# Plonky3/Plonky3-recursion

Hardware: AMD Instinct MI355X
Metric: prove_next_layer ms + Poseidon2 perms/s, KoalaBear 2^20-row circuit, 1/8 GPU (lower is better)
Workload: dtype u32 Montgomery (31-bit prime field, degree-4 extension); Poseidon2 hashing as exact integers in f64; 1 GPU; prove_next_layer (verifier-circuit run on the device + prove_all_tables) of the synthetic koala-bear 2^20-row recursion layer: tables const/public/alu/poseidon2/recompose, FRI blowup 4, arity<=4, 54 queries, 15-bit PoW; circuit inputs + NextLayerPrepCache resident in HBM; field=koala-bear, log_height=20, independent_proofs=1, proof_bytes=612900, parallelism=1 independent proofs, one per GPU, no data-path collective

## Files before the change

plonky3_recursion_amd/csrc/context.h:

```cpp
#pragma once
#include <hip/hip_runtime.h>

#include <algorithm>
#include <array>
#include <atomic>
#include <cstdarg>
#include <cstdio>
#include <cstring>
#include <exception>
#include <functional>
#include <map>
#include <memory>
#include <chrono>
#include <mutex>
#include <stdexcept>
#include <string>
#include <thread>
#include <tuple>
#include <vector>

#include "../../include/p3r.h"
#include "field.h"
#include "poseidon2.h"
#include "proof_layout.h"
// ... 298 lines not shown
  void end_proof() { in_proof = false; }
  HostPost() = default;
  HostPost(const HostPost&) = delete;
  HostPost& operator=(const HostPost&) = delete;
  ~HostPost() {
    if (host) (void)hipHostFree(host);
  }
  hipError_t post(hipStream_t s, const uint32_t* src, size_t words, const uint32_t** out) {
    if (!host) {
      hipError_t e = hipHostMalloc(reinterpret_cast<void**>(&host), (kWords + 16) * 4,
                                   hipHostMallocMapped | hipHostMallocCoherent);
      if (e != hipSuccess) return e;
      e = hipHostGetDevicePointer(reinterpret_cast<void**>(&dev), host, 0);
      if (e != hipSuccess) {
        (void)hipHostFree(host);
        host = nullptr;
        dev = nullptr;
        return e;
      }
      host[kWords] = 0;
    }
    *out = host;
    ++seq;
    hipLaunchKernelGGL(k_post_small, dim3(1), dim3(256), 0, s, dev, src, (uint32_t)words, dev + kWords, seq);
    hipError_t e = hipGetLastError();
    if (e != hipSuccess) return e;
    volatile uint32_t* flag = host + kWords;
    const int sl = slot < kSlots ? slot : kSlots - 1;
    if (in_proof) ++slot;
    const auto t0 = std::chrono::steady_clock::now();
    auto elapsed_ns = [&] { return (int64_t)std::chrono::duration_cast<std::chrono::nanoseconds>(std::chrono::steady_clock::now() - t0).count(); };
    const int64_t expect = in_proof ? expect_ns[sl] : 0;
    if (expect > 400000) {
      const int64_t until = expect - std::max<int64_t>(expect / 4, 200000);
      for (int64_t now = elapsed_ns(); now < until && *flag != seq; now = elapsed_ns())
        std::this_thread::sleep_for(std::chrono::nanoseconds(std::min<int64_t>(until - now, 500000)));
    }
    const int64_t awake_until = expect > 400000 ? expect + expect / 2 + 500000 : 0;
    for (uint64_t spins = 0;; ++spins) {
      if (*flag == seq) break;
      if (spins > (uint64_t(1) << 14) && (spins & 0x3F) == 0x3F) {
        if (awake_until && elapsed_ns() < awake_until) std::this_thread::yield();
        else if (spins > (uint64_t(1) << 17)) std::this_thread::sleep_for(std::chrono::microseconds(20));
        else std::this_thread::yield();
      }
      if ((spins & 0xFFF) == 0xFFF) {
        e = hipStreamQuery(s);
        if (e != hipErrorNotReady) {
          if (e != hipSuccess) return e;
          if (*flag == seq) break;
          return hipStreamSynchronize(s);
        }
      }
    }
    if (in_proof) expect_ns[sl] = elapsed_ns();
    std::atomic_thread_fence(std::memory_order_acquire);
    return hipSuccess;
  }
};

struct DevBuf {
  uint32_t* p = nullptr;
  size_t n = 0;
  std::shared_ptr<DevPool> pool;
  DevBuf() = default;
  explicit DevBuf(size_t cells) { alloc(cells); }
  DevBuf(const DevBuf&) = delete;
  DevBuf& operator=(const DevBuf&) = delete;
  DevBuf(DevBuf&& o) noexcept : p(o.p), n(o.n), pool(std::move(o.pool)) { o.p = nullptr; o.n = 0; }
  DevBuf& operator=(DevBuf&& o) noexcept {
    if (this != &o) { release(); p = o.p; n = o.n; pool = std::move(o.pool); o.p = nullptr; o.n = 0; }
    return *this;
  }
  ~DevBuf() { release(); }
  void alloc(size_t cells) {
    release();
    if (cells) {
      pool = tls_pool();
      if (!pool) fail(P3R_EINVAL, "device allocation outside a p3r API call");
      p = static_cast<uint32_t*>(pool->get(cells * sizeof(uint32_t)));
    }
    n = cells;
  }
  void release() {
    if (p) pool->put(p, n * sizeof(uint32_t));
    p = nullptr;
    n = 0;
    pool.reset();
  }
};

inline int log2_exact(size_t x, const char* what) {
  if (x == 0 || (x & (x - 1))) fail(P3R_EINVAL, "%s (%zu) must be a power of two", what, x);
  int l = 0;
  while ((size_t(1) << l) < x) ++l;
  return l;
}

}

struct p3r_dmat {
  p3r::DevBuf buf;
  uint32_t* d = nullptr;
  size_t h = 0, w = 0;
};

struct p3r_p2_dev {
  size_t n = 0;
  std::unique_ptr<p3r_dmat> inputs;
  p3r::DevBuf flags;
  p3r::DevBuf seed;
};

struct p3r_tree {
  std::vector<const p3r_dmat*> mats;
  std::vector<std::unique_ptr<p3r_dmat>> owned;
  int salt_elems = 0;
  std::vector<std::unique_ptr<p3r_dmat>> salt_owned;
  p3r::DevBuf phase_salts;
  size_t phase_salt_stride = 0, phase_rows = 0;
  int log_max_h = 0;
  int cap_height = 0;
  size_t total_width = 0;
  std::vector<p3r::DevBuf> layers;
  int arity = 2;
  std::vector<p3r::MmcsLevel> levels;
  std::vector<size_t> layer_n;
};

namespace p3r {
struct ProfRec {
  const char* name;
  hipEvent_t a, b;
};
}

struct p3r_ctx {
  p3r_config cfg{};
  std::shared_ptr<p3r::DevPool> pool = std::make_shared<p3r::DevPool>();
  bool prof_enabled = false;
  std::vector<p3r::ProfRec> prof;
  std::vector<std::pair<std::string, double>> stage_ms;
  std::string cur_stage;
  double cur_stage_t0 = 0;
  int partial_rounds = 0;
  hipStream_t stream = nullptr;
  int n_cus = 256;
  p3r::DevBuf rc;
  p3r::DevBuf rc_f64;
  const double* rcd() const { return reinterpret_cast<const double*>(rc_f64.p); }
  size_t rcd_w32_at = 0;
  const double* rcd_w32() const { return rcd() + rcd_w32_at; }
  p3r::DevBuf p2_diag;
  std::vector<uint32_t> rc_canonical;
  std::vector<uint8_t> fri_log_arities;
  p3r::ProofLayout proof_layout;
  std::vector<uint32_t> rc_mont_host;
  std::string err;
  bool w32_diag_builtin = false;
  bool w32_unacknowledged = false;
  uint64_t zk_nonce = 0;
  uint32_t zk_key[8] = {0, 0, 0, 0, 0, 0, 0, 0};
  std::vector<uint8_t> pending_proof;
  p3r::HostStage stage;
  p3r::HostLanding landing;
  p3r::HostPost post;
  std::map<std::string, p3r::DevBuf> const_tables;

  std::map<std::pair<int, int>, p3r::DevBuf> tw_sub;
  std::map<std::pair<int, int>, std::pair<p3r::DevBuf, p3r::DevBuf>> tw4;
  std::map<std::tuple<int, int, uint32_t>, std::pair<p3r::DevBuf, p3r::DevBuf>> pre;
  std::map<std::pair<int, uint32_t>, std::pair<p3r::DevBuf, p3r::DevBuf>> inv_pow;
};

inline hipError_t fetch_small(p3r_ctx* ctx, const uint32_t* src, size_t words, uint32_t* dst) {
  if (words == 0) return hipSuccess;
  if (words <= p3r::HostPost::kWords) {
    const uint32_t* got = nullptr;
    p3r::host_mark("fetch: posted, waiting for the GPU");
    hipError_t e = ctx->post.post(ctx->stream, src, words, &got);
    p3r::host_mark("fetch: arrived");
    if (e != hipSuccess) return e;
    std::memcpy(dst, got, words * 4);
    return hipSuccess;
  }
  return p3r::copy_sync(ctx->stream, dst, src, words * 4, hipMemcpyDeviceToHost);
}
```

plonky3_recursion_amd/csrc/kernels_coop.hip.h:

```cpp
#pragma once
#include "kernels.hip.h"

namespace p3r {

template <int CTRL>
__device__ __forceinline__ uint32_t dpp(uint32_t v) {
  return (uint32_t)__builtin_amdgcn_update_dpp(0, (int)v, CTRL, 0xF, 0xF, false);
}
constexpr int DPP_QUAD_NEXT1 = 0x39;
constexpr int DPP_QUAD_NEXT2 = 0x4E;
constexpr int DPP_QUAD_NEXT3 = 0x93;
constexpr int DPP_ROW_ROR1 = 0x121, DPP_ROW_ROR2 = 0x122, DPP_ROW_ROR4 = 0x124, DPP_ROW_ROR8 = 0x128;

template <class F>
__device__ __forceinline__ F coop_external(F x) {
  F b = F::raw(dpp<DPP_QUAD_NEXT1>(x.v)), c = F::raw(dpp<DPP_QUAD_NEXT2>(x.v)), d = F::raw(dpp<DPP_QUAD_NEXT3>(x.v));
  F ab = x + b;
  F y = ab.dbl() + b + (c + d);
  F t = y + F::raw(dpp<DPP_ROW_ROR4>(y.v));
  t = t + F::raw(dpp<DPP_ROW_ROR8>(t.v));
  return y + t;
}
template <class F>
__device__ __forceinline__ F coop_row_sum(F x) {
  F t = x + F::raw(dpp<DPP_ROW_ROR8>(x.v));
  t = t + F::raw(dpp<DPP_ROW_ROR4>(t.v));
  t = t + F::raw(dpp<DPP_ROW_ROR2>(t.v));
  return t + F::raw(dpp<DPP_ROW_ROR1>(t.v));
}

constexpr int DPP_QUAD_BCAST0 = 0x00;
__device__ __forceinline__ uint32_t coop_bcast0(uint32_t x0) {
  uint32_t q = dpp<DPP_QUAD_BCAST0>(x0);
  q |= dpp<DPP_ROW_ROR4>(q);
  return q | dpp<DPP_ROW_ROR8>(q);
}

template <class PP>
struct CoopRc {
  uint32_t full[2 * P2_HALF_FULL];
  uint32_t part[PP::PARTIAL_ROUNDS];
};
template <class PP>
__device__ __forceinline__ CoopRc<PP> coop_load_rc(const uint32_t* __restrict__ rc, int elem) {
  CoopRc<PP> c;
#pragma unroll
  for (int r = 0; r < P2_HALF_FULL; ++r) c.full[r] = rc[r * P2_WIDTH + elem];
#pragma unroll
  for (int r = 0; r < PP::PARTIAL_ROUNDS; ++r) c.part[r] = rc[P2_HALF_FULL * P2_WIDTH + r];
#pragma unroll
  for (int r = 0; r < P2_HALF_FULL; ++r)
    c.full[P2_HALF_FULL + r] = rc[P2_HALF_FULL * P2_WIDTH + PP::PARTIAL_ROUNDS + r * P2_WIDTH + elem];
  return c;
}

template <class PP>
__device__ __forceinline__ Fp<PP> coop_permute(Fp<PP> s, int elem, Fp<PP> diag, const CoopRc<PP>& rc) {
  using F = Fp<PP>;
  s = coop_external(s);
#pragma unroll
  for (int r = 0; r < P2_HALF_FULL; ++r) {
    s = p2_sbox<PP>(s + F::raw(rc.full[r]));
    s = coop_external(s);
  }
#pragma unroll
  for (int r = 0; r < PP::PARTIAL_ROUNDS; ++r) {
    const F rest = coop_row_sum(elem == 0 ? F::zero() : s);
    const F sb = p2_sbox<PP>(s + F::raw(rc.part[r]));
    const F sum = rest + F::raw(coop_bcast0(elem == 0 ? sb.v : 0u));
    s = (elem == 0 ? sb : s) * diag + sum;
  }
#pragma unroll
  for (int r = 0; r < P2_HALF_FULL; ++r) {
    s = p2_sbox<PP>(s + F::raw(rc.full[P2_HALF_FULL + r]));
    s = coop_external(s);
  }
  return s;
}

template <class PP>
__global__ void __launch_bounds__(kBlock)
k_mmcs_hash_rows_strided_coop(const uint32_t* const* __restrict__ cols, int wtot, size_t h, size_t stride,
                              uint32_t* __restrict__ dig, const uint32_t* __restrict__ rc,
                              const uint32_t* __restrict__ diag) {
  using F = Fp<PP>;
  const size_t gid = (size_t)blockIdx.x * kBlock + threadIdx.x;
  const size_t row = gid >> 4;
  const int e = (int)(gid & 15);
  const bool live = row < h;
  const F d = F::raw(diag[e]);
  const CoopRc<PP> rcs = coop_load_rc<PP>(rc, e);
  F s = F::zero();
  for (int g = 0; g < wtot; g += P2_RATE) {
    if (live && e < P2_RATE && g + e < wtot) s = F::raw(cols[g + e][row * stride]);
    s = coop_permute<PP>(s, e, d, rcs);
  }
  if (live && e < P2_DIGEST) dig[(size_t)e * h + row] = s.v;
}

constexpr int kSubtreeBlock = 1024;
constexpr int kSubtreeNodes = 256;
constexpr int kSubtreeLevels = 8;
struct SubtreeArgs {
  const uint32_t* in;
  uint32_t n_in;
  uint32_t local;
  int n_levels;
  uint32_t* out[kSubtreeLevels];
  const uint32_t* inj[kSubtreeLevels];
  uint32_t* t_state;
  uint32_t* t_beta;
  uint32_t* t_cap;
  int t_dc;
};

template <class PP>
__device__ __forceinline__ void fri_transcript_step(int j, uint32_t root_word, uint32_t* __restrict__ state,
                                                    uint32_t* __restrict__ beta_out, uint32_t* __restrict__ cap_out,
                                                    const CoopRc<PP>& rc, const uint32_t* __restrict__ diag, int dc = 4) {
  using F = Fp<PP>;
  F s = j < P2_RATE ? F::raw(root_word) : F::raw(state[j]);
  if (j < P2_RATE) cap_out[j] = s.v;
  if (j == P2_RATE) s += F::from_canonical(P2_RATE);
  s = coop_permute<PP>(s, j, F::raw(diag[j]), rc);
  state[j] = s.v;
  if (j >= P2_RATE - dc && j < P2_RATE) beta_out[7 - j] = s.v;
}
template <class PP>
__global__ void __launch_bounds__(kSubtreeBlock)
k_mmcs_subtree(SubtreeArgs a, const uint32_t* __restrict__ rc, const uint32_t* __restrict__ diag) {
  using F = Fp<PP>;
  __shared__ uint32_t buf[2][P2_DIGEST * kSubtreeNodes / 2];
  const int elem = threadIdx.x & 15;
  const uint32_t group = threadIdx.x >> 4, k = elem & 7;
  const F d = F::raw(diag[elem]);
  const CoopRc<PP> rcs = coop_load_rc<PP>(rc, elem);
  uint32_t n = a.n_in < a.local ? a.n_in : a.local;
  uint32_t n_glob = a.n_in, first = blockIdx.x * n;
#pragma unroll
  for (int l = 0; l < kSubtreeLevels; ++l) {
    if (l < a.n_levels) {
      const uint32_t nn = n / 2, nn_glob = n_glob / 2, first_out = first / 2;
      const uint32_t* cur = buf[(l + 1) & 1];
      uint32_t* nxt = buf[l & 1];
      for (uint32_t node = group; node < nn; node += blockDim.x / 16) {
        const uint32_t child = 2 * node + (elem >> 3);
        F s = F::raw(l == 0 ? a.in[(size_t)k * n_glob + first + child] : cur[k * n + child]);
        s = coop_permute<PP>(s, elem, d, rcs);
        if (a.inj[l]) {
          if (elem >= P2_DIGEST) s = F::raw(a.inj[l][(size_t)k * nn_glob + first_out + node]);
          s = coop_permute<PP>(s, elem, d, rcs);
        }
        if (elem < P2_DIGEST) {
          nxt[k * nn + node] = s.v;
          a.out[l][(size_t)k * nn_glob + first_out + node] = s.v;
        }
      }
      __syncthreads();
      n = nn;
      n_glob = nn_glob;
      first = first_out;
    }
  }
  if (a.t_state && threadIdx.x < P2_WIDTH) {
    const uint32_t* root = buf[(a.n_levels - 1) & 1];
    fri_transcript_step<PP>((int)threadIdx.x, threadIdx.x < P2_RATE ? root[threadIdx.x] : 0u, a.t_state, a.t_beta,
                            a.t_cap, rcs, diag, a.t_dc ? a.t_dc : 4);
  }
}

template <class PP>
__global__ void __launch_bounds__(64)
k_fri_transcript_step(const uint32_t* __restrict__ root , uint32_t* __restrict__ state ,
                      uint32_t* __restrict__ beta_out , uint32_t* __restrict__ cap_out ,
                      const uint32_t* __restrict__ rc, const uint32_t* __restrict__ diag, int dc) {
  const int j = threadIdx.x;
  if (j >= P2_WIDTH) return;
  fri_transcript_step<PP>(j, j < P2_RATE ? root[j] : 0u, state, beta_out, cap_out, coop_load_rc<PP>(rc, j), diag, dc);
}



template <class F>
__device__ __forceinline__ F coop32_pair_sum(F t) {
  const auto r = __builtin_amdgcn_permlane16_swap(t.v, t.v, false, false);
  return F::raw(r[0]) + F::raw(r[1]);
}
template <class F>
__device__ __forceinline__ F coop32_external(F x) {
  const F b = F::raw(dpp<DPP_QUAD_NEXT1>(x.v)), c = F::raw(dpp<DPP_QUAD_NEXT2>(x.v)), d = F::raw(dpp<DPP_QUAD_NEXT3>(x.v));
  const F ab = x + b;
  const F y = ab.dbl() + b + (c + d);
  F t = y + F::raw(dpp<DPP_ROW_ROR4>(y.v));
  t = t + F::raw(dpp<DPP_ROW_ROR8>(t.v));
  return y + coop32_pair_sum(t);
}
template <class F>
__device__ __forceinline__ F coop32_sum(F x) { return coop32_pair_sum(coop_row_sum(x)); }
__device__ __forceinline__ uint32_t coop32_bcast0(uint32_t x0) {
  const uint32_t q = coop_bcast0(x0);
  const auto r = __builtin_amdgcn_permlane16_swap(q, q, false, false);
  return r[0] | r[1];
}

template <class PP>
struct Coop32Rc {
  uint32_t full[2 * P2_HALF_FULL];
  uint32_t part[PP::PARTIAL_ROUNDS_W32];
  uint32_t diag;
};
template <class PP>
__device__ __forceinline__ Coop32Rc<PP> coop32_load_rc(const uint32_t* __restrict__ rcw, int elem) {
  Coop32Rc<PP> c;
#pragma unroll
  for (int r = 0; r < P2_HALF_FULL; ++r) c.full[r] = rcw[r * P2W_WIDTH + elem];
#pragma unroll
  for (int r = 0; r < PP::PARTIAL_ROUNDS_W32; ++r) c.part[r] = rcw[P2_HALF_FULL * P2W_WIDTH + r];
#pragma unroll
  for (int r = 0; r < P2_HALF_FULL; ++r)
    c.full[P2_HALF_FULL + r] = rcw[P2_HALF_FULL * P2W_WIDTH + PP::PARTIAL_ROUNDS_W32 + r * P2W_WIDTH + elem];
  c.diag = rcw[p2w_num_rc<PP>() + elem];
  return c;
}
template <class PP>
__device__ __forceinline__ Fp<PP> coop32_permute(Fp<PP> s, int elem, const Coop32Rc<PP>& rc) {
  using F = Fp<PP>;
  const F diag = F::raw(rc.diag);
  s = coop32_external(s);
#pragma unroll
  for (int r = 0; r < P2_HALF_FULL; ++r) {
    s = p2_sbox<PP>(s + F::raw(rc.full[r]));
    s = coop32_external(s);
  }
#pragma unroll 1
  for (int r = 0; r < PP::PARTIAL_ROUNDS_W32; ++r) {
    const F rest = coop32_sum(elem == 0 ? F::zero() : s);
    const F sb = p2_sbox<PP>(s + F::raw(rc.part[r]));
    const F sum = rest + F::raw(coop32_bcast0(elem == 0 ? sb.v : 0u));
    s = (elem == 0 ? sb : s) * diag + sum;
  }
#pragma unroll
  for (int r = 0; r < P2_HALF_FULL; ++r) {
    s = p2_sbox<PP>(s + F::raw(rc.full[P2_HALF_FULL + r]));
    s = coop32_external(s);
  }
  return s;
}

}
```

plonky3_recursion_amd/csrc/mmcs_impl.hip.h:

```cpp

namespace {

template <class PP>
void hash_rows(p3r_ctx* ctx, const std::vector<std::vector<const p3r_dmat*>>& classes,
               const std::vector<uint32_t*>& digs) {
  std::vector<HashRowsJob> jobs;
  for (size_t c = 0; c < classes.size(); ++c) {
    std::vector<const uint32_t*> cols;
    for (const p3r_dmat* m : classes[c])
      for (size_t k = 0; k < m->w; ++k) cols.push_back(m->d + k * m->h);
    HashRowsJob j{};
    j.cols = col_table(ctx, cols);
    j.dig = digs[c];
    j.h = classes[c][0]->h;
    j.wtot = (int)cols.size();
    jobs.push_back(j);
  }
  std::stable_sort(jobs.begin(), jobs.end(),
                   [](const HashRowsJob& a, const HashRowsJob& b) { return a.wtot > b.wtot; });
  uint32_t blocks = 0;
  double perms = 0;
  for (auto& j : jobs) {
    j.block0 = blocks;
    blocks += blocks_for(j.h);
    perms += (double)j.h * ((j.wtot + P2_RATE - 1) / P2_RATE);
  }
  prof_count(ctx, "hash_rows_perms", perms);
  const auto* d_jobs =
      static_cast<const HashRowsJob*>(const_table(ctx, jobs.data(), jobs.size() * sizeof(HashRowsJob)));
  ProfScope ps(ctx, "mmcs_hash_rows");
  hipLaunchKernelGGL(k_mmcs_hash_rows<PP>, dim3(blocks), dim3(kBlock), 0, ctx->stream, d_jobs, (int)jobs.size(),
                     ctx->rcd());
  P3R_HIP(hipGetLastError());
}

inline size_t env_pow2(const char* name, size_t dflt, size_t lo, size_t hi) {
  const char* e = tuning_knob(name);
  size_t v = e ? (size_t)atol(e) : dflt;
  v = std::min(std::max(v, lo), hi);
  while (v & (v - 1)) v &= v - 1;
  return v;
}
inline size_t coop_max_nodes() {
  static const size_t v = env_pow2("P3R_COOP_MAX_NODES", 16384, 1, size_t(1) << 30);
  return v;
}
inline size_t coop_max_leaf_rows() {
  static const size_t v = env_pow2("P3R_COOP_MAX_LEAF_ROWS", 8192, 1, size_t(1) << 30);
  return v;
}
inline size_t subtree_nodes() {
  static const size_t v = env_pow2("P3R_SUBTREE_NODES", 32, 2, kSubtreeNodes);
  return v;
}
template <class PP>
void launch_compress(p3r_ctx* ctx, const uint32_t* prev, const uint32_t* inj, uint32_t* out, size_t n) {
  ProfScope ps(ctx, "mmcs_compress");
  hipLaunchKernelGGL(k_mmcs_compress<PP>, dim3(blocks_for(n)), dim3(kBlock), 0, ctx->stream, prev, inj, out, n,
                     ctx->rcd());
  P3R_HIP(hipGetLastError());
}

using InjectMap = std::map<size_t, DevBuf>;
inline const uint32_t* injected_at(const InjectMap* inject, const MmcsLevel& lv) {
  if (!lv.inject_h) return nullptr;
  if (!inject || !inject->count(lv.inject_h) || lv.inject_h != lv.logical_next)
    fail(P3R_EINVAL, "MMCS: matrix heights must be powers of two");
  return inject->at(lv.inject_h).p;
}
inline void push_layer(p3r_tree* tree, size_t n) {
  tree->layers.emplace_back(P2_DIGEST * n);
  tree->layer_n.push_back(n);
}

struct TranscriptStep {
  uint32_t *state, *beta, *cap;
  bool done = false;
  int dc = 4;
};
template <class PP>
size_t mmcs_subtree(p3r_ctx* ctx, p3r_tree* tree, size_t l, const InjectMap* inject, TranscriptStep* step) {
  const size_t n = tree->layer_n.back();
  if (n / 2 > coop_max_nodes()) return 0;
  SubtreeArgs a{};
  a.in = tree->layers.back().p;
  a.n_in = (uint32_t)n;
  const size_t local = std::min<size_t>(n, subtree_nodes());
  a.local = (uint32_t)local;
  for (size_t shrink = local; shrink > 1 && l + a.n_levels < tree->levels.size() && a.n_levels < kSubtreeLevels; shrink /= 2) {
    const MmcsLevel& lv = tree->levels[l + a.n_levels];
    push_layer(tree, lv.padded_next);
    a.out[a.n_levels] = tree->layers.back().p;
    a.inj[a.n_levels] = injected_at(inject, lv);
    ++a.n_levels;
  }
  if (step && tree->layer_n.back() == 1 && n == local) {
    a.t_state = step->state;
    a.t_beta = step->beta;
    a.t_cap = step->cap;
    a.t_dc = step->dc;
    step->done = true;
  }
  ProfScope ps(ctx, "mmcs_compress");
  const unsigned lanes = (unsigned)std::min<size_t>(std::max<size_t>(local * 8, 64), kSubtreeBlock);
  hipLaunchKernelGGL(k_mmcs_subtree<PP>, dim3((unsigned)(n / local)), dim3(lanes), 0, ctx->stream, a,
                     ctx->rc.p, ctx->p2_diag.p);
  P3R_HIP(hipGetLastError());
  return (size_t)a.n_levels;
}

inline void mmcs_begin(p3r_ctx* ctx, p3r_tree* tree, const std::vector<size_t>& heights) {
  const size_t hmax = *std::max_element(heights.begin(), heights.end());
  tree->arity = ctx->cfg.mmcs_arity == 4 ? 4 : 2;
  tree->log_max_h = log2_exact(hmax, "matrix height");
  tree->cap_height = (int)ctx->cfg.cap_height;
  tree->levels = tree->arity == 4 ? mmcs4_schedule(heights) : mmcs2_schedule(heights, tree->log_max_h, tree->cap_height);
  tree->layers.clear();
  tree->layer_n.clear();
  const size_t n0 = tree->arity == 4 ? mmcs4_padded_len(hmax) : hmax;
  push_layer(tree, n0);
  if (n0 != hmax) P3R_HIP(fill_async(ctx->stream, tree->layers[0].p, 0, P2_DIGEST * n0 * 4));
}

template <class PP>
void mmcs_build_levels(p3r_ctx* ctx, p3r_tree* tree, const InjectMap* inject, TranscriptStep* step = nullptr) {
  for (size_t l = 0; l < tree->levels.size();) {
    if (tree->arity != 4) {
      const size_t built = mmcs_subtree<PP>(ctx, tree, l, inject, step);
      if (built) {
        l += built;
        continue;
      }
    }
    const MmcsLevel& lv = tree->levels[l++];
    DevBuf next(P2_DIGEST * lv.padded_next);
    const uint32_t* inj = injected_at(inject, lv);
    if (tree->arity == 4)
      mmcs4_compress<PP>(ctx, tree->layers.back().p, tree->layer_n.back(), lv.step, inj, next.p, lv.logical_next, lv.padded_next);
    else
      launch_compress<PP>(ctx, tree->layers.back().p, inj, next.p, lv.padded_next);
    tree->layers.push_back(std::move(next));
    tree->layer_n.push_back(lv.padded_next);
  }
}

template <class PP>
void mmcs_hash_rows_strided(p3r_ctx* ctx, p3r_tree* tree, const std::vector<const uint32_t*>& cols, size_t rows, size_t stride) {
  const uint32_t* const* dcols = col_table(ctx, cols);
  uint32_t* dig = tree->layers[0].p;
  if (tree->arity == 4) {
    mmcs4_hash_rows_strided<PP>(ctx, dcols, (int)cols.size(), rows, stride, dig, tree->layer_n[0]);
  } else {
    ProfScope ps(ctx, "mmcs_hash_rows_strided");
    if (rows <= coop_max_leaf_rows())
      hipLaunchKernelGGL(k_mmcs_hash_rows_strided_coop<PP>, dim3(blocks_for(rows * 16)), dim3(kBlock), 0,
                         ctx->stream, dcols, (int)cols.size(), rows, stride, dig, ctx->rc.p, ctx->p2_diag.p);
    else
      hipLaunchKernelGGL(k_mmcs_hash_rows_strided<PP>, dim3(blocks_for(rows)), dim3(kBlock), 0, ctx->stream,
                         dcols, (int)cols.size(), rows, stride, dig, ctx->rcd());
  }
  P3R_HIP(hipGetLastError());
}

inline std::vector<uint32_t> mmcs_cap_mont(p3r_ctx* ctx, const p3r_tree* tree) {
  const size_t cap_n = tree->layer_n.back();
  std::vector<uint32_t> soa(P2_DIGEST * cap_n), cap(P2_DIGEST * cap_n);
  P3R_HIP(fetch_small(ctx, tree->layers.back().p, soa.size(), soa.data()));
  for (size_t j = 0; j < cap_n; ++j)
    for (int k = 0; k < P2_DIGEST; ++k) cap[j * P2_DIGEST + k] = soa[(size_t)k * cap_n + j];
  return cap;
}

template <class PP>
std::vector<uint32_t> mmcs_commit(p3r_ctx* ctx, p3r_tree* tree) {
  const auto& mats = tree->mats;
  if (mats.empty()) fail(P3R_EINVAL, "MMCS commit needs at least one matrix");
  std::vector<size_t> order(mats.size()), heights, class_h;
  std::iota(order.begin(), order.end(), 0);
  std::stable_sort(order.begin(), order.end(),
                   [&](size_t a, size_t b) { return mats[a]->h > mats[b]->h; });
  const size_t hmax = mats[order[0]]->h;
  const int log_max_h = log2_exact(hmax, "matrix height");
  if ((int)ctx->cfg.cap_height > log_max_h)
    fail(P3R_EINVAL, "cap_height %d exceeds log2 of the tallest matrix (%d)", (int)ctx->cfg.cap_height, log_max_h);
  tree->total_width = 0;
  for (auto* m : mats) {
    tree->total_width += m->w;
    heights.push_back(m->h);
  }
  mmcs_begin(ctx, tree, heights);
  for (size_t i : order)
    if (class_h.empty() || class_h.back() != mats[i]->h) class_h.push_back(mats[i]->h);
  InjectMap inject;
  {
    std::vector<std::vector<const p3r_dmat*>> classes;
    std::vector<uint32_t*> digs;
    std::vector<size_t> allocs;
    for (size_t h : class_h) {
      std::vector<const p3r_dmat*> v;
      for (size_t i : order)
        if (mats[i]->h == h) v.push_back(mats[i]);
      classes.push_back(std::move(v));
      digs.push_back(h == hmax ? tree->layers[0].p : inject.emplace(h, DevBuf(P2_DIGEST * h)).first->second.p);
      allocs.push_back(h == hmax ? tree->layer_n[0] : h);
    }
    if (tree->arity == 4) mmcs4_hash_rows<PP>(ctx, classes, digs, allocs);
    else hash_rows<PP>(ctx, classes, digs);
  }
  mmcs_build_levels<PP>(ctx, tree, &inject);
  return mmcs_cap_mont(ctx, tree);
}

template <class PP>
void mmcs_open(p3r_ctx* ctx, const p3r_tree* tree, size_t index, uint32_t* opened, uint32_t* proof) {
  using F = Fp<PP>;
  if (index >> tree->log_max_h) fail(P3R_EINVAL, "open index %zu out of range", index);
  size_t off = 0;
  for (const p3r_dmat* m : tree->mats) {
    int lh = log2_exact(m->h, "matrix height");
    size_t row = index >> (tree->log_max_h - lh);
    P3R_HIP(hipMemcpy2DAsync(opened + off, 4, m->d + row, m->h * 4, 4, m->w, hipMemcpyDeviceToHost,
                             ctx->stream));
    off += m->w;
  }
  size_t depth = 0;
  for (size_t l = 0; l < tree->levels.size(); ++l) {
    const size_t step = tree->levels[l].step, idx = index >> tree->levels[l].bits, pos = idx & (step - 1);
    for (size_t j = 0; j < step; ++j) {
      if (j == pos) continue;
      P3R_HIP(hipMemcpy2DAsync(proof + depth * P2_DIGEST, 4, tree->layers[l].p + (idx - pos + j), tree->layer_n[l] * 4, 4,
                               P2_DIGEST, hipMemcpyDeviceToHost, ctx->stream));
      ++depth;
    }
  }
  P3R_HIP(hipStreamSynchronize(ctx->stream));
  for (size_t i = 0; i < off; ++i) opened[i] = F::raw(opened[i]).to_canonical();
  for (size_t i = 0; i < depth * P2_DIGEST; ++i) proof[i] = F::raw(proof[i]).to_canonical();
}

struct OpenItem {
  const uint32_t* base;
  uint64_t n;
  uint32_t dst;
  uint32_t shift;
  uint32_t step, slot;
};
template <class PP>
__global__ void __launch_bounds__(256)
k_mmcs_open_batch(const OpenItem* __restrict__ items, uint32_t n_items, const uint32_t* __restrict__ indices, uint32_t words,
// ... 72 lines not shown
```

plonky3_recursion_amd/csrc/p3r_core.hip:

```cpp
#include "context.h"
#include "kernels.hip.h"
#include "kernels_stark.hip.h"
#include "kernels_coop.hip.h"
#include "tu_api.h"
#include "profile.h"
#include "run_schedule.h"
#include "prep_device.h"
#include "host_abi.h"

#include <sys/random.h>

#include <algorithm>
#include <cerrno>
#include <future>
#include <numeric>
#include <unordered_map>

using namespace p3r;

namespace {

thread_local std::string g_create_error;

template <class Fn>
// ... 136 lines not shown
  hipLaunchKernelGGL(k_p2w_permute_rows<PP>, dim3(blocks_for(n)), dim3(kBlock), 0, ctx->stream, d, n, ctx->rc.p + p2_num_constants<PP>());
  P3R_HIP(hipGetLastError());
}

template <class PP>
std::unique_ptr<p3r_dmat> coset_lde(p3r_ctx* ctx, const p3r_dmat* in, int added_bits, uint32_t shift) {
  return std::move(coset_lde_batch<PP>(ctx, {{in, shift}}, added_bits)[0]);
}

template <class PP>
void init_ctx(p3r_ctx* ctx) {
  using F = Fp<PP>;
  const size_t nrc = p2_num_constants<PP>();
  const std::vector<uint32_t> table = constants_table<PP>(ctx->cfg, [](const char* what, uint32_t got, size_t want) {
    fail(P3R_EINVAL, "%s is %u, the field needs %zu constants", what, got, want);
  });
  const uint32_t* src = table.data();
  ctx->rc_canonical = table;
  std::vector<uint32_t> mont(table.size());
  for (size_t i = 0; i < table.size(); ++i) {
    if (table[i] >= PP::P) fail(P3R_EINVAL, "permutation constant %zu is not canonical", i);
    mont[i] = F::from_canonical(table[i]).v;
  }
  ctx->rc_mont_host = mont;
  ctx->rc.alloc(mont.size());
  P3R_HIP(copy_sync(ctx->stream, ctx->rc.p, mont.data(), mont.size() * 4, hipMemcpyHostToDevice));
  std::vector<double> rcd(src, src + nrc);
  ctx->rcd_w32_at = nrc;
  {
    const size_t nrcw = p2w_num_rc<PP>();
    const uint32_t* w = src + nrc;
    rcd.insert(rcd.end(), w, w + nrcw);
    for (int i = 0; i < P2W_WIDTH; ++i) {
      const uint32_t d = w[nrcw + i];
      rcd.push_back(d > PP::P / 2 ? (double)d - (double)PP::P : (double)d);
    }
    const uint32_t* builtin = PP::FIELD_ID == 0 ? kDefaultDiagW32_koala_bear : kDefaultDiagW32_baby_bear;
    const bool is_builtin = std::equal(builtin, builtin + P2W_WIDTH, w + nrcw) && !tuning_knob("P3R_W32_GENERAL_DIAG");
    ctx->w32_diag_builtin = is_builtin;
  }
  ctx->rc_f64.alloc(2 * rcd.size());
  P3R_HIP(copy_sync(ctx->stream, ctx->rc_f64.p, rcd.data(), rcd.size() * 8, hipMemcpyHostToDevice));
  {
    auto inv2k = [](int k) { return F::from_u64(uint64_t(1) << k).inv(); };
    const F two = F::from_canonical(2), three = F::from_canonical(3), four = F::from_canonical(4);
    F d[16] = {-two, F::one(), two, inv2k(1), three, four, -inv2k(1), -three, -four, inv2k(8), inv2k(3), inv2k(24),
               -inv2k(8), -inv2k(3), -inv2k(4), -inv2k(24)};
    if (PP::FIELD_ID == 1) {
      F b[16] = {-two, F::one(), two, inv2k(1), three, four, -inv2k(1), -three, -four, inv2k(8), inv2k(2), inv2k(3),
                 inv2k(27), -inv2k(8), -inv2k(4), -inv2k(27)};
      for (int i = 0; i < 16; ++i) d[i] = b[i];
    }
    uint32_t dm[16];
    for (int i = 0; i < 16; ++i) dm[i] = d[i].v;
    ctx->p2_diag.alloc(16);
    P3R_HIP(copy_sync(ctx->stream, ctx->p2_diag.p, dm, sizeof dm, hipMemcpyHostToDevice));
  }
  ctx->partial_rounds = PP::PARTIAL_ROUNDS;
  ctx->cfg.poseidon2_rc = nullptr;
  ctx->w32_unacknowledged = (!ctx->cfg.poseidon2_w32_rc || !ctx->cfg.poseidon2_w32_diag) && !(ctx->cfg.ext_choices & P3R_EXT_UNPINNED_W32_DEFAULTS);
  if (ctx->w32_unacknowledged && ctx->cfg.mmcs_arity == 4)
    fail(P3R_EINVAL, "mmcs_arity = 4 with poseidon2_w32_rc / poseidon2_w32_diag NULL: the built-in width-32 constants are self-generated, "
                     "not upstream's - pass the caller's, or acknowledge with P3R_EXT_UNPINNED_W32_DEFAULTS");
  ctx->cfg.poseidon2_w32_rc = nullptr;
  ctx->cfg.poseidon2_w32_diag = nullptr;
  if (ctx->cfg.fri_log_arities) ctx->fri_log_arities.assign(ctx->cfg.fri_log_arities, ctx->cfg.fri_log_arities + ctx->cfg.fri_log_arities_len);
  ctx->cfg.fri_log_arities = nullptr;
  if (!ctx->proof_layout.set(ctx->cfg.proof_layout, ctx->cfg.proof_layout_len))
    fail(P3R_EINVAL, "proof_layout must be 18 bytes: three permutations batch[5] | fri[5] | opened[8]");
  ctx->cfg.proof_layout = nullptr;
  lde_init<PP>(ctx);
}

}

#include "mmcs_impl.hip.h"
#include "prove_impl.hip.h"
#include "layer_impl.hip.h"
#include "circuit_impl.hip.h"

namespace {
template <class PP>
void mmcs_commit_canonical(p3r_ctx* ctx, p3r_tree* tree, uint32_t* cap_out) {
  const size_t S = ctx->cfg.mmcs_salt_elems, n_mats = tree->mats.size();
  if (S) {
    const std::vector<const p3r_dmat*> mats = tree->mats;
    for (const p3r_dmat* m : mats) log2_exact(m->h, "matrix height");
    const ZkKey key = zk_key_of(ctx, ctx->zk_nonce++);
    tree->salt_elems = (int)S;
    tree->salt_owned = draw_salts<PP>(ctx, mats, kSaltRound + ZK_ROUND_PUBLIC_COMMIT, key);
    tree->mats.clear();
    for (size_t i = 0; i < n_mats; ++i) { tree->mats.push_back(mats[i]); tree->mats.push_back(tree->salt_owned[i].get()); }
  }
  const std::vector<uint32_t> cap = mmcs_commit<PP>(ctx, tree);
  tree->total_width -= n_mats * S;
  for (size_t i = 0; i < cap.size(); ++i) cap_out[i] = Fp<PP>::raw(cap[i]).to_canonical();
}
}

extern "C" {

p3r_ctx* p3r_create(const p3r_config* cfg) {
  p3r_ctx* ctx = nullptr;
  int rc = guard(nullptr, [&] {
    if (!cfg) fail(P3R_EINVAL, "cfg is NULL");
    if (cfg->abi_version != P3R_ABI_VERSION)
      fail(P3R_EINVAL, "abi_version %u != %u", cfg->abi_version, P3R_ABI_VERSION);
    if (cfg->field != P3R_FIELD_KOALA_BEAR && cfg->field != P3R_FIELD_BABY_BEAR)
      fail(P3R_EUNSUPPORTED, "unsupported field id %u", cfg->field);
    if (cfg->mmcs_arity != 0 && cfg->mmcs_arity != 2 && cfg->mmcs_arity != 4)
      fail(P3R_EINVAL, "mmcs_arity must be 2 or 4 (got %u)", cfg->mmcs_arity);
    if (cfg->mmcs_arity == 4 && cfg->cap_height != 0) fail(P3R_EUNSUPPORTED, "arity-4 MMCS: cap_height must be 0");
    if (cfg->zk > 1) fail(P3R_EINVAL, "zk must be 0 or 1 (got %u)", cfg->zk);
    if (cfg->zk && cfg->num_random_codewords > 8) fail(P3R_EINVAL, "num_random_codewords must be in 1..8 (0 selects 2)");
    if (cfg->challenge_degree != 0 && cfg->challenge_degree != 4 &&
        !(cfg->challenge_degree == 5 && cfg->field == P3R_FIELD_KOALA_BEAR))
      fail(P3R_EUNSUPPORTED, "UnsupportedChallengeDegree(%u): 4, or 5 over KoalaBear", cfg->challenge_degree);
    if (p3r::ext_degree_is_binomial_generic(cfg->ext_degree)) {
      const uint32_t P = cfg->field == P3R_FIELD_KOALA_BEAR ? p3r::KoalaBearParams::P : p3r::BabyBearParams::P;
      if (cfg->ext_w == 0 || cfg->ext_w >= P) fail(P3R_EINVAL, "MissingWForExtension: ext_degree %u needs ext_w in 1..p-1", cfg->ext_degree);
    } else if (cfg->ext_degree != 1 && cfg->ext_degree != 4 && !(cfg->ext_degree == 5 && cfg->field == P3R_FIELD_KOALA_BEAR))
      fail(P3R_EUNSUPPORTED, "UnsupportedExtDegree(%u): 1, 2, 4, 6, 8, or 5 over KoalaBear", cfg->ext_degree);
    int ndev = 0;
    hipError_t e = hipGetDeviceCount(&ndev);
    if (e != hipSuccess || ndev == 0)
      fail(P3R_ENODEV, "no HIP device available (%s); this library has no CPU fallback",
           e == hipSuccess ? "device count is 0" : hipGetErrorString(e));
    if (cfg->device < 0 || cfg->device >= ndev)
      fail(P3R_ENODEV, "device %d out of range (%d devices)", cfg->device, ndev);
    P3R_HIP(hipSetDevice(cfg->device));
    auto c = std::make_unique<p3r_ctx>();
    c->cfg = *cfg;
    tls_pool() = c->pool;
    P3R_HIP(hipStreamCreateWithFlags(&c->stream, hipStreamNonBlocking));
    {
      int cus = 0;
      if (hipDeviceGetAttribute(&cus, hipDeviceAttributeMultiprocessorCount, cfg->device) == hipSuccess && cus > 0) c->n_cus = cus;
    }
    if (cfg->mmcs_salt_elems > 16) fail(P3R_EINVAL, "mmcs_salt_elems must be in 0..16 (got %u)", cfg->mmcs_salt_elems);
    if (cfg->zk || cfg->mmcs_salt_elems) {
      uint32_t entropy[4] = {0, 0, 0, 0};
      const bool deterministic = cfg->ext_choices & P3R_EXT_ZK_DETERMINISTIC;
      if (!deterministic) {
        size_t got = 0;
        while (got < sizeof entropy) {
          const ssize_t r = getrandom(reinterpret_cast<uint8_t*>(entropy) + got, sizeof entropy - got, 0);
          if (r < 0) { if (errno == EINTR) continue; fail(P3R_EHIP, "getrandom failed (errno %d): no entropy for the ZK key", errno); }
          got += (size_t)r;
        }
      }
      zk_context_key(cfg->zk_key, entropy, deterministic, c->zk_key);
    }
    P3R_FIELD_CALL(c, init_ctx, c.get());
    ctx = c.release();
  });
  return rc == P3R_OK ? ctx : nullptr;
}

void p3r_destroy(p3r_ctx* ctx) {
  if (!ctx) return;
  (void)hipSetDevice(ctx->cfg.device);
  (void)hipStreamSynchronize(ctx->stream);
  prof_clear(ctx);
  (void)hipStreamDestroy(ctx->stream);
  std::shared_ptr<DevPool> pool = ctx->pool;
  delete ctx;
  pool->trim();
  if (tls_pool() == pool) tls_pool().reset();
}

const char* p3r_last_error(const p3r_ctx* ctx) {
  return ctx ? ctx->err.c_str() : g_create_error.c_str();
}

uint32_t p3r_poseidon2_trace_width(const p3r_ctx* ctx) {
  return ctx->cfg.field == P3R_FIELD_KOALA_BEAR ? p2_perm_cols<KoalaBearParams>() + 2
                                                : p2_perm_cols<BabyBearParams>() + 2;
}
uint32_t p3r_poseidon2_num_constants(const p3r_ctx* ctx) {
  return ctx->cfg.field == P3R_FIELD_KOALA_BEAR ? p2_num_constants<KoalaBearParams>()
                                                : p2_num_constants<BabyBearParams>();
}
int p3r_poseidon2_round_constants(const p3r_ctx* ctx, uint32_t* out) {
  if (!ctx || !out) return P3R_EINVAL;
  std::copy(ctx->rc_canonical.begin(), ctx->rc_canonical.begin() + p3r_poseidon2_num_constants(ctx), out);
  return P3R_OK;
}

uint64_t p3r_zk_nonce(const p3r_ctx* ctx) { return ctx ? ctx->zk_nonce : 0; }
int p3r_zk_set_nonce(p3r_ctx* ctx, uint64_t nonce) {
  if (!ctx) return P3R_EINVAL;
  if (!(ctx->cfg.ext_choices & P3R_EXT_ZK_DETERMINISTIC)) {
    ctx->err = "p3r_zk_set_nonce needs P3R_EXT_ZK_DETERMINISTIC: replaying a nonce repeats the masks of an earlier proof";
    return P3R_EINVAL;
  }
  ctx->zk_nonce = nonce;
  return P3R_OK;
}

int p3r_trim(p3r_ctx* ctx, uint64_t* freed_bytes) {
  if (!ctx) return P3R_EINVAL;
  return guard(ctx, [&] {
    P3R_HIP(hipStreamSynchronize(ctx->stream));
    if (freed_bytes) {
      std::lock_guard<std::mutex> g(ctx->pool->mu);
      *freed_bytes = ctx->pool->cached_bytes;
    }
    ctx->pool->trim();
    ctx->const_tables.clear();
  });
}

int p3r_sync(p3r_ctx* ctx) {
  return guard(ctx, [&] { P3R_HIP(hipStreamSynchronize(ctx->stream)); });
}

p3r_dmat* p3r_dmat_upload(p3r_ctx* ctx, const uint32_t* rowmajor, size_t h, size_t w) {
  p3r_dmat* out = nullptr;
  guard(ctx, [&] {
    if (!rowmajor) fail(P3R_EINVAL, "rowmajor is NULL");
    out = P3R_FIELD_CALL(ctx, upload, ctx, rowmajor, h, w).release();
  });
  return out;
}
p3r_dmat* p3r_dmat_alloc(p3r_ctx* ctx, size_t h, size_t w) {
  p3r_dmat* out = nullptr;
  guard(ctx, [&] { out = dmat_alloc(h, w).release(); });
  return out;
}
int p3r_dmat_download(p3r_ctx* ctx, const p3r_dmat* m, uint32_t* out) {
  return guard(ctx, [&] {
    if (!m || !out) fail(P3R_EINVAL, "NULL argument");
    P3R_FIELD_CALL(ctx, download, ctx, m, out);
  });
}
size_t p3r_dmat_height(const p3r_dmat* m) { return m->h; }
size_t p3r_dmat_width(const p3r_dmat* m) { return m->w; }
void p3r_dmat_free(p3r_ctx* ctx, p3r_dmat* m) {
  if (ctx) (void)hipStreamSynchronize(ctx->stream);
  delete m;
}

int p3r_poseidon2_permute_dmat(p3r_ctx* ctx, p3r_dmat* states) {
  return guard(ctx, [&] {
    if (!states) fail(P3R_EINVAL, "states is NULL");
    P3R_FIELD_CALL(ctx, permute_dmat, ctx, states);
  });
}

int p3r_poseidon2_permute_batch(p3r_ctx* ctx, const uint32_t* in, uint32_t* out, size_t n) {
  return guard(ctx, [&] {
    if (!in || !out) fail(P3R_EINVAL, "NULL argument");
    if (n == 0) return;
    size_t np = 1;
    while (np < n) np <<= 1;
    std::vector<uint32_t> padded;
    const uint32_t* src = in;
    if (np != n) {
      padded.assign(np * P2_WIDTH, 0);
      memcpy(padded.data(), in, n * P2_WIDTH * 4);
      src = padded.data();
    }
    auto m = P3R_FIELD_CALL(ctx, upload, ctx, src, np, (size_t)P2_WIDTH);
    P3R_FIELD_CALL(ctx, permute_dmat, ctx, m.get());
    if (np != n) {
      P3R_FIELD_CALL(ctx, download, ctx, m.get(), padded.data());
      memcpy(out, padded.data(), n * P2_WIDTH * 4);
    } else {
      P3R_FIELD_CALL(ctx, download, ctx, m.get(), out);
    }
  });
}

p3r_p2_dev* p3r_p2_rows_upload(p3r_ctx* ctx, const p3r_p2_rows* rows) {
  p3r_p2_dev* out = nullptr;
  guard(ctx, [&] {
    if (!rows) fail(P3R_EINVAL, "rows is NULL");
    out = P3R_FIELD_CALL(ctx, p2_rows_upload, ctx, rows).release();
  });
  return out;
}
void p3r_p2_rows_free(p3r_ctx* ctx, p3r_p2_dev* rows) {
  if (ctx) (void)hipStreamSynchronize(ctx->stream);
  delete rows;
}
p3r_dmat* p3r_poseidon2_trace_fill_dev(p3r_ctx* ctx, const p3r_p2_dev* rows) {
  p3r_dmat* out = nullptr;
  guard(ctx, [&] {
    if (!rows) fail(P3R_EINVAL, "rows is NULL");
    out = P3R_FIELD_CALL(ctx, trace_fill, ctx, rows).release();
  });
  return out;
}
p3r_dmat* p3r_poseidon2_trace_fill_dmat(p3r_ctx* ctx, const p3r_p2_rows* rows) {
  p3r_dmat* out = nullptr;
  guard(ctx, [&] {
    if (!rows) fail(P3R_EINVAL, "rows is NULL");
    auto d = P3R_FIELD_CALL(ctx, p2_rows_upload, ctx, rows);
    out = P3R_FIELD_CALL(ctx, trace_fill, ctx, d.get()).release();
  });
  return out;
}

int p3r_poseidon2_trace_fill(p3r_ctx* ctx, const p3r_p2_rows* rows, uint32_t* trace_out) {
  return guard(ctx, [&] {
    if (!rows || !trace_out) fail(P3R_EINVAL, "NULL argument");
// ... 463 lines not shown
```

Measured before the change: 26.13 ms.

## Fuse Merkle subtree levels across workgroups with last-arriver atomic counters

The Merkle subtree kernel now reduces all levels in a single launch. When a workgroup finishes its local subtree, it bumps an arrival counter, and the last workgroup of each group carries on to the higher levels after an acquire/release fence. This removes the separate kernel launches per 8-level chunk, along with their host round trips, and allows the FRI transcript step to be fused even when the tree spans several workgroups. In exchange, the upper levels run serially in a single workgroup with low parallelism, and correctness now depends on the counter reset and on memory-fence ordering.

After: 26.51 ms. +1.4%, slower.

```diff
diff --git a/plonky3_recursion_amd/csrc/context.h b/plonky3_recursion_amd/csrc/context.h
--- a/plonky3_recursion_amd/csrc/context.h
+++ b/plonky3_recursion_amd/csrc/context.h
@@ -474,6 +474,7 @@
   size_t rcd_w32_at = 0;
   const double* rcd_w32() const { return rcd() + rcd_w32_at; }
   p3r::DevBuf p2_diag;
+  p3r::DevBuf subtree_counters;
   std::vector<uint32_t> rc_canonical;
   std::vector<uint8_t> fri_log_arities;
   p3r::ProofLayout proof_layout;
diff --git a/plonky3_recursion_amd/csrc/kernels_coop.hip.h b/plonky3_recursion_amd/csrc/kernels_coop.hip.h
--- a/plonky3_recursion_amd/csrc/kernels_coop.hip.h
+++ b/plonky3_recursion_amd/csrc/kernels_coop.hip.h
@@ -100,7 +100,7 @@
 
 constexpr int kSubtreeBlock = 1024;
 constexpr int kSubtreeNodes = 256;
-constexpr int kSubtreeLevels = 8;
+constexpr int kSubtreeLevels = 16;
 struct SubtreeArgs {
   const uint32_t* in;
   uint32_t n_in;
@@ -108,6 +108,7 @@
   int n_levels;
   uint32_t* out[kSubtreeLevels];
   const uint32_t* inj[kSubtreeLevels];
+  uint32_t* counters;
   uint32_t* t_state;
   uint32_t* t_beta;
   uint32_t* t_cap;
@@ -131,40 +132,67 @@
 k_mmcs_subtree(SubtreeArgs a, const uint32_t* __restrict__ rc, const uint32_t* __restrict__ diag) {
   using F = Fp<PP>;
   __shared__ uint32_t buf[2][P2_DIGEST * kSubtreeNodes / 2];
+  __shared__ uint32_t carry;
   const int elem = threadIdx.x & 15;
   const uint32_t group = threadIdx.x >> 4, k = elem & 7;
   const F d = F::raw(diag[elem]);
   const CoopRc<PP> rcs = coop_load_rc<PP>(rc, elem);
-  uint32_t n = a.n_in < a.local ? a.n_in : a.local;
-  uint32_t n_glob = a.n_in, first = blockIdx.x * n;
-#pragma unroll
-  for (int l = 0; l < kSubtreeLevels; ++l) {
-    if (l < a.n_levels) {
+  const uint32_t* src = a.in;
+  uint32_t n_glob = a.n_in;
+  uint32_t wg = blockIdx.x;
+  uint32_t cnt_at = 0;
+  int lvl = 0;
+  const uint32_t* top = buf[0];
+  for (;;) {
+    uint32_t n = n_glob < a.local ? n_glob : a.local;
+    const uint32_t n_wgs = n_glob / n;
+    uint32_t first = wg * n;
+#pragma unroll 1
+    for (int l = 0; n > 1 && lvl < a.n_levels; ++l, ++lvl) {
       const uint32_t nn = n / 2, nn_glob = n_glob / 2, first_out = first / 2;
       const uint32_t* cur = buf[(l + 1) & 1];
       uint32_t* nxt = buf[l & 1];
+      uint32_t* out = a.out[lvl];
+      const uint32_t* inj = a.inj[lvl];
       for (uint32_t node = group; node < nn; node += blockDim.x / 16) {
         const uint32_t child = 2 * node + (elem >> 3);
-        F s = F::raw(l == 0 ? a.in[(size_t)k * n_glob + first + child] : cur[k * n + child]);
+        F s = F::raw(l == 0 ? src[(size_t)k * n_glob + first + child] : cur[k * n + child]);
         s = coop_permute<PP>(s, elem, d, rcs);
-        if (a.inj[l]) {
-          if (elem >= P2_DIGEST) s = F::raw(a.inj[l][(size_t)k * nn_glob + first_out + node]);
+        if (inj) {
+          if (elem >= P2_DIGEST) s = F::raw(inj[(size_t)k * nn_glob + first_out + node]);
           s = coop_permute<PP>(s, elem, d, rcs);
         }
         if (elem < P2_DIGEST) {
           nxt[k * nn + node] = s.v;
-          a.out[l][(size_t)k * nn_glob + first_out + node] = s.v;
+          out[(size_t)k * nn_glob + first_out + node] = s.v;
         }
       }
+      if (nn == 1 && n_wgs > 1 && lvl + 1 < a.n_levels && threadIdx.x < 64)
+        __builtin_amdgcn_fence(__ATOMIC_RELEASE, "agent");
       __syncthreads();
       n = nn;
       n_glob = nn_glob;
       first = first_out;
+      top = nxt;
     }
-  }
-  if (a.t_state && threadIdx.x < P2_WIDTH) {
-    const uint32_t* root = buf[(a.n_levels - 1) & 1];
-    fri_transcript_step<PP>((int)threadIdx.x, threadIdx.x < P2_RATE ? root[threadIdx.x] : 0u, a.t_state, a.t_beta,
+    if (lvl >= a.n_levels || n_wgs == 1) break;
+    const uint32_t members = n_wgs < a.local ? n_wgs : a.local;
+    const uint32_t grp = wg / members;
+    if (threadIdx.x == 0) {
+      uint32_t* c = a.counters + cnt_at + grp;
+      const bool last = atomicAdd(c, 1u) == members - 1;
+      if (last) *c = 0;
+      carry = last;
+    }
+    __syncthreads();
+    if (!carry) return;
+    __builtin_amdgcn_fence(__ATOMIC_ACQUIRE, "agent");
+    src = a.out[lvl - 1];
+    cnt_at += n_wgs / members;
+    wg = grp;
+  }
+  if (a.t_state && n_glob == 1 && threadIdx.x < P2_WIDTH) {
+    fri_transcript_step<PP>((int)threadIdx.x, threadIdx.x < P2_RATE ? top[threadIdx.x] : 0u, a.t_state, a.t_beta,
                             a.t_cap, rcs, diag, a.t_dc ? a.t_dc : 4);
   }
 }
diff --git a/plonky3_recursion_amd/csrc/mmcs_impl.hip.h b/plonky3_recursion_amd/csrc/mmcs_impl.hip.h
--- a/plonky3_recursion_amd/csrc/mmcs_impl.hip.h
+++ b/plonky3_recursion_amd/csrc/mmcs_impl.hip.h
@@ -78,6 +78,19 @@
   bool done = false;
   int dc = 4;
 };
+inline size_t subtree_counters(size_t n, size_t local) {
+  size_t total = 0;
+  for (size_t wgs = n / std::min(n, local); wgs > 1;) {
+    wgs /= std::min(wgs, local);
+    total += wgs;
+  }
+  return total;
+}
+inline void subtree_counters_init(p3r_ctx* ctx) {
+  const size_t words = std::max<size_t>(subtree_counters(2 * coop_max_nodes(), subtree_nodes()), 1);
+  ctx->subtree_counters.alloc(words);
+  P3R_HIP(fill_async(ctx->stream, ctx->subtree_counters.p, 0, words * 4));
+}
 template <class PP>
 size_t mmcs_subtree(p3r_ctx* ctx, p3r_tree* tree, size_t l, const InjectMap* inject, TranscriptStep* step) {
   const size_t n = tree->layer_n.back();
@@ -87,14 +100,16 @@
   a.n_in = (uint32_t)n;
   const size_t local = std::min<size_t>(n, subtree_nodes());
   a.local = (uint32_t)local;
-  for (size_t shrink = local; shrink > 1 && l + a.n_levels < tree->levels.size() && a.n_levels < kSubtreeLevels; shrink /= 2) {
+  for (size_t shrink = n; shrink > 1 && l + a.n_levels < tree->levels.size() && a.n_levels < kSubtreeLevels; shrink /= 2) {
     const MmcsLevel& lv = tree->levels[l + a.n_levels];
     push_layer(tree, lv.padded_next);
     a.out[a.n_levels] = tree->layers.back().p;
     a.inj[a.n_levels] = injected_at(inject, lv);
     ++a.n_levels;
   }
-  if (step && tree->layer_n.back() == 1 && n == local) {
+  if (subtree_counters(n, local) > ctx->subtree_counters.n) fail(P3R_EHIP, "internal: Merkle arrival counters too few for %zu digests", n);
+  a.counters = ctx->subtree_counters.p;
+  if (step && tree->layer_n.back() == 1) {
     a.t_state = step->state;
     a.t_beta = step->beta;
     a.t_cap = step->cap;
diff --git a/plonky3_recursion_amd/csrc/p3r_core.hip b/plonky3_recursion_amd/csrc/p3r_core.hip
--- a/plonky3_recursion_amd/csrc/p3r_core.hip
+++ b/plonky3_recursion_amd/csrc/p3r_core.hip
@@ -312,6 +312,7 @@
       zk_context_key(cfg->zk_key, entropy, deterministic, c->zk_key);
     }
     P3R_FIELD_CALL(c, init_ctx, c.get());
+    subtree_counters_init(c.get());
     ctx = c.release();
   });
   return rc == P3R_OK ? ctx : nullptr;
```
